# ooowedyn/InkLayer

Hardware: AMD Instinct MI355X
Metric: sketches/sec end-to-end (GroundingDINO+SAM) at 1024x1024 (higher is better)
Workload: dtype f16 (MFMA, f32 accumulate; f32 residual/norm/softmax; split-f16 = fp32-grade operands for patch-embed, neck, mask decoder); 1 GPU; full GroundingDINO Swin-T + SAM ViT-H pipeline, batch=8 per GPU, 1024x1024 synthetic sketches, 16 boxes/sketch, random-init weights; global_batch=8, parallelism=image-parallel x1

## Files before the change

inklayer_amd/csrc/attention.hip:

```cpp
#include <stdlib.h>
#include "mfma_util.h"
#include "../../include/inklayer_hip.h"

int ink_win4_attn_launch(const InkAttn& p, int n_cus, hipStream_t s);
int ink_glob4_attn_launch(const InkAttn& p, hipStream_t s);

namespace {

__device__ __forceinline__ f16x8 cvt8(const f32x16& s, int base) {
  f16x8 r;
#pragma unroll
  for (int j = 0; j < 8; ++j) r[j] = (f16)s[base + j];
  return r;
}

template <int HD, int MODE, int NW, bool ALLKV = false>
__global__ __launch_bounds__(NW * 64) void flash_attn_kernel(InkAttn p) {
  constexpr int NQKB = HD / 16;
  constexpr int NQK = NQKB + (MODE == 2 ? 2 : 0);
  constexpr int NB = (HD + 31) / 32;
  constexpr int DVP = NB * 32;
  constexpr bool LSUM_MFMA = DVP >= HD + 8;
  constexpr int CH = HD / 8;
  constexpr int KROW = ((NQK * 2) | 1) * 16;
// ... 319 lines not shown
    };
    if constexpr (LSUM_MFMA && !ALLKV) {
#pragma unroll
      for (int r = 0; r < 16; ++r) s0[r] = __builtin_amdgcn_exp2f(fmaf(s0[r], c, koff));
      pf[0] = cvt8(s0, 0);
      pf[1] = cvt8(s0, 8);
      if (half) {
#pragma unroll
        for (int ks = 0; ks < 2; ++ks)
#pragma unroll
          for (int i = 0; i < NB; ++i) pv(ks, i);
      } else {
        constexpr int NG = 2 * NB;
#pragma unroll
        for (int g = 0; g < NG; ++g) {
          pv(g / NB, g % NB);
#pragma unroll
          for (int r = (16 * g) / NG; r < (16 * (g + 1)) / NG; ++r) s1[r] = __builtin_amdgcn_exp2f(fmaf(s1[r], c, koff));
        }
        pf[2] = cvt8(s1, 0);
        pf[3] = cvt8(s1, 8);
#pragma unroll
        for (int ks = 2; ks < 4; ++ks)
#pragma unroll
          for (int i = 0; i < NB; ++i) pv(ks, i);
      }
    } else {
      float ps = 0.f;
#pragma unroll
      for (int r = 0; r < 16; ++r) {
        s0[r] = __builtin_amdgcn_exp2f(fmaf(s0[r], c, koff));
        s1[r] = __builtin_amdgcn_exp2f(fmaf(s1[r], c, koff));
        ps += s0[r] + s1[r];
      }
      if constexpr (!LSUM_MFMA) l_run += ps;
      pf[0] = cvt8(s0, 0);
      pf[1] = cvt8(s0, 8);
      pf[2] = cvt8(s1, 0);
      pf[3] = cvt8(s1, 8);
#pragma unroll
      for (int ks = 0; ks < 4; ++ks) {
        if (ks >= 2 && half) break;
#pragma unroll
        for (int i = 0; i < NB; ++i) pv(ks, i);
      }
    }
    if constexpr (!ALLKV) {
      if (t + 1 < ntiles) {
        store_tile(t + 1);
        if (t + 2 < ntiles) load_tile(t + 2);
      }
      __syncthreads();
    }
  }

  float ltot;
  if constexpr (LSUM_MFMA) {
    ltot = o[LI][LR];
  } else {
    ltot = l_run + __shfl_xor(l_run, 32, 64);
  }
  const float inv = 1.0f / ltot;
  if (q_ok) {
    const int64_t o_row = (MODE == 2 && ALLKV && p.tok_rows) ? q_row : (int64_t)b * p.n_q + q_idx;
    f16* Orow = (f16*)p.O + o_row * p.ldo + h * HD;
#pragma unroll
    for (int i = 0; i < NB; ++i)
#pragma unroll
      for (int g = 0; g < 4; ++g) {
        const int d0 = 32 * i + 8 * g + 4 * hh;
        if (d0 < HD) {
          const f16x4 v = {(f16)(o[i][4 * g] * inv), (f16)(o[i][4 * g + 1] * inv),
                           (f16)(o[i][4 * g + 2] * inv), (f16)(o[i][4 * g + 3] * inv)};
          *(f16x4*)(Orow + d0) = v;
        }
      }
  }
  if constexpr (ALLKV) {
    if (blk + 1 < blk_end) qs = load_q(blk + 1, qf);
  }
  }
}

template <int HD, int S, bool AUG, bool F16T = false>
__global__ __launch_bounds__(256) void relpos_mfma_kernel(const f16* __restrict__ Q, int64_t ldq,
                                                          const float* __restrict__ Rh,
                                                          const float* __restrict__ Rw, int n_heads,
                                                          float inv_scale, const int32_t* __restrict__ tok_rows,
                                                          float* __restrict__ out_h, float* __restrict__ out_w,
                                                          f16* __restrict__ out_aug) {
  constexpr int NQ = S * S;
  constexpr int RT = (2 * S - 1 + 31) / 32;
  constexpr int ROWS = 2 * RT * 32;
  constexpr int TROW = (HD / 8 + 1) * 16;
  constexpr int NQG = (NQ + 31) / 32;
  constexpr int GPB = AUG ? NQG : 8;
  constexpr int OROW = (AUG ? 64 : 256) + 16;
  __shared__ __attribute__((aligned(16))) char tab[ROWS * TROW + 4 * 32 * OROW];
  const int tid = threadIdx.x, lane = tid & 63, wave = tid >> 6;
  const int lq = lane & 31, hh = lane >> 5;
  char* ot = tab + ROWS * TROW + wave * 32 * OROW;
  const int nblk = (NQG + GPB - 1) / GPB;
  const int bh = blockIdx.x / nblk, gb = blockIdx.x % nblk;
  const int b = bh / n_heads, h = bh % n_heads;
  for (int i = tid; i < ROWS * (HD / 8); i += 256) {
    const int r = i / (HD / 8), c8 = i % (HD / 8);
    const int tr = r % (RT * 32);
    const float* src = (r < RT * 32 ? Rh : Rw) + (int64_t)tr * HD + c8 * 8;
    f16x8 v = {0, 0, 0, 0, 0, 0, 0, 0};
    if (tr < 2 * S - 1) {
      const f32x4 a = *(const f32x4*)src, c = *(const f32x4*)(src + 4);
      v = (f16x8){(f16)a[0], (f16)a[1], (f16)a[2], (f16)a[3], (f16)c[0], (f16)c[1], (f16)c[2], (f16)c[3]};
    }
    *(f16x8*)(tab + r * TROW + c8 * 16) = v;
  }
  __syncthreads();
  for (int g = gb * GPB + wave; g < min(NQG, (gb + 1) * GPB); g += 4) {
    const int q = g * 32 + lq;
    bool q_ok = q < NQ;
    const int qc = q_ok ? q : NQ - 1;
    int64_t qrow = (int64_t)b * NQ + qc;
    if (AUG && tok_rows) {
      const int r = tok_rows[qrow];
      q_ok = q_ok && r >= 0;
      qrow = r >= 0 ? r : 0;
    }
    const f16* qp = Q + qrow * ldq + h * HD;
    f16x8 qf[HD / 16];
#pragma unroll
    for (int s = 0; s < HD / 16; ++s) qf[s] = *(const f16x8*)(qp + 16 * s + 8 * hh);
    const int qh = qc / S, qw = qc % S;
    if (AUG && hh == 0) *(f16x4*)(ot + lq * OROW + 56) = (f16x4){0, 0, 0, 0};
#pragma unroll
    for (int tt = 0; tt < 2 * RT; ++tt) {
      f32x16 d;
#pragma unroll
      for (int r = 0; r < 16; ++r) d[r] = 0.f;
#pragma unroll
      for (int s = 0; s < HD / 16; ++s) {
        const f16x8 a = *(const f16x8*)(tab + (tt * 32 + lq) * TROW + (2 * s + hh) * 16);
        d = mfma32(a, qf[s], d);
      }
      const bool is_w = tt >= RT;
      const int base = (is_w ? qw : qh) + S - 1 - (tt % RT) * 32;
#pragma unroll
      for (int r = 0; r < 16; ++r) {
        const int j = base - ((r & 3) + 8 * (r >> 2) + 4 * hh);
        if (j >= 0 && j < S) {
          const float v = d[r] * inv_scale;
          if (AUG) {
            *(f16*)(ot + lq * OROW + ((is_w ? S : 0) + j) * 2) = (f16)v;
          } else {
            *(float*)(ot + lq * OROW + j * 4) = v;
          }
        }
      }
      if (!AUG && (tt % RT) == RT - 1) {
        if (F16T) {
          f16* dst = (f16*)(is_w ? out_w : out_h) + ((int64_t)bh * NQ + q) * S + hh * 32;
          if (q_ok) {
#pragma unroll
            for (int i = 0; i < 4; ++i) {
              const f32x4 a = *(const f32x4*)(ot + lq * OROW + hh * 128 + i * 32), c = *(const f32x4*)(ot + lq * OROW + hh * 128 + i * 32 + 16);
              *(f16x8*)(dst + 8 * i) = (f16x8){(f16)a[0], (f16)a[1], (f16)a[2], (f16)a[3], (f16)c[0], (f16)c[1], (f16)c[2], (f16)c[3]};
            }
          }
        } else {
          float* dst = (is_w ? out_w : out_h) + ((int64_t)bh * NQ + q) * S + hh * 32;
          if (q_ok) {
#pragma unroll
            for (int i = 0; i < 8; ++i) *(f32x4*)(dst + 4 * i) = *(const f32x4*)(ot + lq * OROW + hh * 128 + i * 16);
          }
        }
      }
    }
    if (AUG && q_ok) {
      f16* dst = out_aug + ((int64_t)bh * NQ + q) * 32 + hh * 16;
      *(f16x8*)dst = *(const f16x8*)(ot + lq * OROW + hh * 32);
      *(f16x8*)(dst + 8) = *(const f16x8*)(ot + lq * OROW + hh * 32 + 16);
    }
  }
}

}

extern "C" int ink_flash_attn(const InkAttn* pp, void* stream) {
  INK_CHECK_ARG(pp != nullptr);
  const InkAttn& p = *pp;
  INK_CHECK_ARG(p.Q && p.K && p.V && p.O);
  INK_CHECK_ARG(p.n_batch > 0 && p.n_heads > 0 && p.n_q > 0 && p.n_k > 0);
  INK_CHECK_ARG(p.ldq % 8 == 0 && p.ldk % 8 == 0 && p.ldv % 8 == 0 && p.ldo % 4 == 0);
  INK_CHECK_ARG(ink_aligned<16>(p.Q, p.K, p.V) && ink_aligned<8>(p.O));
  INK_CHECK_ARG(!p.tok_rows || p.bias_mode == 2);
  static const int n_cus = [] {
    int dev = 0, n = 0;
    if (hipGetDevice(&dev) != hipSuccess || hipDeviceGetAttribute(&n, hipDeviceAttributeMultiprocessorCount, dev) != hipSuccess || n <= 0) n = 256;
    return n;
  }();
  constexpr bool persist = true;
  hipStream_t s = (hipStream_t)stream;
  const int bhn = p.n_batch * p.n_heads;
#define INK_FA_X(HD, MODE, NW, ALL)                                                                      \
  {                                                                                                        \
    constexpr int nqk_ = HD / 16 + (MODE == 2 ? 2 : 0);                                                    \
    constexpr int lds_ = (ALL ? 4 : 2) * (64 * (((nqk_ * 2) | 1) * 16) + 64 * (((HD + 31) / 32) * 64)) +   \
                         0;                                                                            \
    ink_dyn_lds<flash_attn_kernel<HD, MODE, NW, ALL>>(lds_);                                               \
    const int nqb = (p.n_q + NW * 32 - 1) / (NW * 32);                                                     \
    const int grid_ = (ALL && persist) ? (bhn * nqb < n_cus ? bhn * nqb : n_cus) : bhn * nqb;                \
    hipLaunchKernelGGL((flash_attn_kernel<HD, MODE, NW, ALL>), dim3(grid_), dim3(NW * 64), lds_, s, p);      \
  }
#define INK_FA(HD, MODE, NW) INK_FA_X(HD, MODE, NW, false)
  if (p.head_dim == 80 && p.bias_mode == 1) {
    INK_CHECK_ARG(p.rel_h && p.rel_w && p.grid_w == 64 && p.n_k % 64 == 0);
    if (p.n_q % 256 == 0 && p.n_k % 128 == 0 && p.n_k >= 256 && p.n_k <= 4096) return ink_glob4_attn_launch(p, s);
    INK_CHECK_ARG(!p.rel_f16);
    INK_FA(80, 1, 8);
  } else if (p.head_dim == 80 && p.bias_mode == 2) {
    INK_CHECK_ARG(p.rel_aug && p.grid_w > 0 && p.grid_w <= 16 && p.n_k <= p.grid_w * p.grid_w && p.n_k <= 256);
    INK_CHECK_ARG(!p.tok_rows || (p.n_q == p.n_k && p.pad_k && p.pad_v &&
                                  ink_aligned<16>(p.pad_k, p.pad_v)));
    if (p.n_k >= 193 && p.n_k <= 208 && p.n_q <= 256 &&
        (p.tok_rows || (int64_t)p.n_batch * p.n_q * p.ldo * 2 < 0x80000000LL))
      return ink_win4_attn_launch(p, n_cus, s);
    INK_FA_X(80, 2, 7, true);
  } else if (p.head_dim == 64 && p.bias_mode == 1) {
    INK_CHECK_ARG(p.rel_h && p.rel_w && p.grid_w == 64 && p.n_k % 64 == 0 && p.n_k <= 64 * 64);
    INK_CHECK_ARG(!p.rel_f16);
    INK_FA(64, 1, 8);
  } else if (p.head_dim == 64 && p.bias_mode == 2) {
    INK_CHECK_ARG(p.rel_aug && p.grid_w > 0 && p.grid_w <= 16 && p.n_k <= p.grid_w * p.grid_w && p.n_k <= 256);
    INK_CHECK_ARG(!p.tok_rows || (p.n_q == p.n_k && p.pad_k && p.pad_v &&
                                  ink_aligned<16>(p.pad_k, p.pad_v)));
    INK_FA_X(64, 2, 7, true);
  } else if (p.head_dim == 80 && p.bias_mode == 0) {
    INK_FA(80, 0, 4);
  } else if (p.head_dim == 64 && p.bias_mode == 0) {
    INK_FA(64, 0, 4);
  } else if (p.head_dim == 32 && p.bias_mode == 0) {
    if (p.n_q <= 32) { INK_FA(32, 0, 1) } else { INK_FA(32, 0, 4) }
  } else if (p.head_dim == 32 && p.bias_mode == 3) {
    INK_CHECK_ARG(p.dense_bias && p.n_k <= 64 && p.n_q <= 64 && (!p.dense_mask || p.n_mask > 0));
    INK_FA(32, 3, 2);
  } else if (p.head_dim == 16 && p.bias_mode == 0) {
    if (p.n_q <= 32) { INK_FA(16, 0, 1) } else { INK_FA(16, 0, 4) }
  } else {
    return INK_ERR_ARG;
  }
#undef INK_FA
#undef INK_FA_X
  return ink_launch_status();
}

extern "C" int ink_relpos_bias64_f16(const void* Q, int64_t ldq, const float* rel_pos_h, const float* rel_pos_w,
                                     int32_t n_batch, int32_t n_heads, int32_t head_dim, float scale, void* out_h_f16,
                                     void* out_w_f16, void* stream) {
  INK_CHECK_ARG(Q && rel_pos_h && rel_pos_w && head_dim == 80 && ldq % 8 == 0 && out_h_f16 && out_w_f16);
  INK_CHECK_ARG(n_batch > 0 && n_heads > 0 && scale > 0.f && ink_aligned<16>(out_h_f16, out_w_f16));
  hipLaunchKernelGGL((relpos_mfma_kernel<80, 64, false, true>), dim3(n_batch * n_heads * 16), dim3(256), 0, (hipStream_t)stream,
                     (const f16*)Q, ldq, rel_pos_h, rel_pos_w, n_heads, 1.0f / scale, (const int32_t*)nullptr,
                     (float*)out_h_f16, (float*)out_w_f16, (f16*)nullptr);
  return ink_launch_status();
}

extern "C" int ink_relpos_bias(const void* Q, int64_t ldq, const float* rel_pos_h,
                               const float* rel_pos_w, int32_t S, int32_t n_batch,
                               int32_t n_heads, int32_t head_dim, float scale, const int32_t* tok_rows,
                               float* out_h, float* out_w, void* out_aug_f16, void* stream) {
  INK_CHECK_ARG(Q && rel_pos_h && rel_pos_w && (head_dim == 80 || head_dim == 64) && ldq % 8 == 0);
  INK_CHECK_ARG(n_batch > 0 && n_heads > 0 && S > 0 && scale > 0.f);
  if (out_aug_f16) {
    INK_CHECK_ARG(S <= 16);
  } else {
    INK_CHECK_ARG(S == 64 && out_h && out_w && !tok_rows);
  }
  const f16* q = (const f16*)Q;
  hipStream_t st = (hipStream_t)stream;
  const int nbh = n_batch * n_heads;
  if (out_aug_f16) {
    INK_CHECK_ARG(S == 14);
    if (head_dim == 80) {
      hipLaunchKernelGGL((relpos_mfma_kernel<80, 14, true>), dim3(nbh), dim3(256), 0, st, q, ldq, rel_pos_h,
                         rel_pos_w, n_heads, 1.0f / scale, tok_rows, out_h, out_w, (f16*)out_aug_f16);
    } else {
      hipLaunchKernelGGL((relpos_mfma_kernel<64, 14, true>), dim3(nbh), dim3(256), 0, st, q, ldq, rel_pos_h,
                         rel_pos_w, n_heads, 1.0f / scale, tok_rows, out_h, out_w, (f16*)out_aug_f16);
    }
  } else if (head_dim == 80) {
    hipLaunchKernelGGL((relpos_mfma_kernel<80, 64, false>), dim3(nbh * 16), dim3(256), 0, st, q, ldq, rel_pos_h,
                       rel_pos_w, n_heads, 1.0f / scale, (const int32_t*)nullptr, out_h, out_w, (f16*)nullptr);
  } else {
    hipLaunchKernelGGL((relpos_mfma_kernel<64, 64, false>), dim3(nbh * 16), dim3(256), 0, st, q, ldq, rel_pos_h,
                       rel_pos_w, n_heads, 1.0f / scale, (const int32_t*)nullptr, out_h, out_w, (f16*)nullptr);
  }
  return ink_launch_status();
}
```

inklayer_amd/csrc/attn_few.hip:

```cpp
#include "common.h"
#include "../../include/inklayer_hip.h"

namespace {

__device__ __forceinline__ void load8(const f16* p, float* d) {
  const f16x8 v = *(const f16x8*)p;
#pragma unroll
  for (int j = 0; j < 8; ++j) d[j] = (float)v[j];
}
__device__ __forceinline__ void load8(const float* p, float* d) {
  const f32x4 a = *(const f32x4*)p, b = *(const f32x4*)(p + 4);
#pragma unroll
  for (int j = 0; j < 4; ++j) { d[j] = a[j]; d[4 + j] = b[j]; }
}
__device__ __forceinline__ void store8(f16* p, const float* d) {
  f16x8 v;
#pragma unroll
  for (int j = 0; j < 8; ++j) v[j] = (f16)d[j];
  *(f16x8*)p = v;
}
__device__ __forceinline__ void store8(float* p, const float* d) {
  *(f32x4*)p = (f32x4){d[0], d[1], d[2], d[3]};
  *(f32x4*)(p + 4) = (f32x4){d[4], d[5], d[6], d[7]};
}

template <int HD, typename T>
__global__ __launch_bounds__(256) void attn_fewkeys_kernel(const T* __restrict__ Q, int64_t ldq,
                                                           const T* __restrict__ K, int64_t ldk,
                                                           const T* __restrict__ V, int64_t ldv, int B,
                                                           int n_q, int n_k, int n_heads, float scale,
                                                           const uint8_t* __restrict__ blocked,
                                                           const int32_t* __restrict__ q_rows,
                                                           const float* __restrict__ q_add,
                                                           T* __restrict__ O, int64_t ldo) {
  const int64_t gid = (int64_t)blockIdx.x * 256 + threadIdx.x;
  if (gid >= (int64_t)B * n_q * n_heads) return;
  const int h = (int)(gid % n_heads);
  const int64_t bq = gid / n_heads;
  const int b = (int)(bq / n_q), q = (int)(bq % n_q);
  float qv[HD];
  const T* qp = Q + (q_rows ? (int64_t)q_rows[b] + q : bq) * ldq + h * HD;
#pragma unroll
  for (int i = 0; i < HD / 8; ++i) load8(qp + 8 * i, qv + 8 * i);
  if (q_add) {
    const float* ap = q_add + ((int64_t)q * n_heads + h) * HD;
#pragma unroll
    for (int i = 0; i < HD; ++i) qv[i] += ap[i];
  }
  float sc[16];
  float mx = -3.0e38f;
  for (int t = 0; t < n_k; ++t) {
    const T* kp = K + ((int64_t)b * n_k + t) * ldk + h * HD;
    float d = 0.f;
#pragma unroll
    for (int i = 0; i < HD / 8; ++i) {
      float kv[8];
      load8(kp + 8 * i, kv);
#pragma unroll
      for (int j = 0; j < 8; ++j) d = fmaf(qv[8 * i + j], kv[j], d);
    }
    d *= scale;
    if (blocked && blocked[q * n_k + t]) d = -3.0e38f;
    sc[t] = d;
    mx = fmaxf(mx, d);
  }
  float sum = 0.f;
  for (int t = 0; t < n_k; ++t) { sc[t] = sc[t] <= -1.0e38f ? 0.f : expf(sc[t] - mx); sum += sc[t]; }
  const float inv = 1.f / sum;
  float acc[HD];
#pragma unroll
  for (int i = 0; i < HD; ++i) acc[i] = 0.f;
  for (int t = 0; t < n_k; ++t) {
    const T* vp = V + ((int64_t)b * n_k + t) * ldv + h * HD;
    const float pw = sc[t] * inv;
#pragma unroll
    for (int i = 0; i < HD / 8; ++i) {
      float vv[8];
      load8(vp + 8 * i, vv);
#pragma unroll
      for (int j = 0; j < 8; ++j) acc[8 * i + j] = fmaf(pw, vv[j], acc[8 * i + j]);
    }
  }
  T* op = O + bq * ldo + h * HD;
#pragma unroll
  for (int i = 0; i < HD / 8; ++i) store8(op + 8 * i, acc + 8 * i);
}


template <int NK>
__global__ __launch_bounds__(256) void attn_fewkeys16_f32_kernel(const float* __restrict__ Q, int64_t ldq,
                                                                 const float* __restrict__ K, int64_t ldk,
                                                                 const float* __restrict__ V, int64_t ldv, int B,
                                                                 int n_q, int n_heads, float scale,
                                                                 const int32_t* __restrict__ q_rows,
                                                                 const float* __restrict__ q_add,
                                                                 float* __restrict__ O, int64_t ldo) {
  const int64_t gid = (int64_t)blockIdx.x * 256 + threadIdx.x;
  if (gid >= (int64_t)B * n_q * n_heads * 4) return;
  const int part = (int)(gid & 3);
  const int h = (int)((gid >> 2) % n_heads);
  const int64_t bq = (gid >> 2) / n_heads;
  const int b = (int)(bq / n_q), q = (int)(bq % n_q);
  const int col = h * 16 + 4 * part;
  f32x4 qv = *(const f32x4*)(Q + (q_rows ? (int64_t)q_rows[b] + q : bq) * ldq + col);
  if (q_add) qv += *(const f32x4*)(q_add + (int64_t)q * n_heads * 16 + col);
  qv *= scale * 1.44269504088896340736f;
  const float* kp = K + (int64_t)b * NK * ldk + col;
  const float* vp = V + (int64_t)b * NK * ldv + col;
  f32x4 kv[NK], vv[NK];
#pragma unroll
  for (int t = 0; t < NK; ++t) {
    kv[t] = *(const f32x4*)(kp + (int64_t)t * ldk);
    vv[t] = *(const f32x4*)(vp + (int64_t)t * ldv);
  }
  float sc[NK];
  float mx = -3.0e38f;
#pragma unroll
  for (int t = 0; t < NK; ++t) {
    float d = (qv[0] * kv[t][0] + qv[1] * kv[t][1]) + (qv[2] * kv[t][2] + qv[3] * kv[t][3]);
    d += __builtin_bit_cast(float, __builtin_amdgcn_update_dpp(0, __builtin_bit_cast(int, d), 0xB1, 0xF, 0xF, false));
    d += __builtin_bit_cast(float, __builtin_amdgcn_update_dpp(0, __builtin_bit_cast(int, d), 0x4E, 0xF, 0xF, false));
    sc[t] = d;
    mx = fmaxf(mx, d);
  }
  float sum = 0.f;
#pragma unroll
  for (int t = 0; t < NK; ++t) { sc[t] = __builtin_amdgcn_exp2f(sc[t] - mx); sum += sc[t]; }
  const float inv = 1.f / sum;
  f32x4 acc = {0.f, 0.f, 0.f, 0.f};
#pragma unroll
  for (int t = 0; t < NK; ++t) acc += (sc[t] * inv) * vv[t];
  *(f32x4*)(O + bq * ldo + col) = acc;
}

template <int QW>
__global__ __launch_bounds__(512) void attn_fewq16_kernel(const float* __restrict__ Q, int64_t ldq,
                                                          const float* __restrict__ K, int64_t ldk,
                                                          const float* __restrict__ V, int64_t ldv, int n_q,
                                                          int n_k, int n_heads, float scale,
                                                          const int32_t* __restrict__ q_rows,
                                                          const int32_t* __restrict__ kv_rows,
                                                          const float* __restrict__ k_add,
                                                          float* __restrict__ O, int64_t ldo) {
  constexpr int KSPLIT = 2, HD = 16, HB = 4, TK = 64;
  constexpr int ROWE = HB * HD;
  constexpr int CH = 4, NCH = ROWE / CH;
  constexpr int NU = TK * NCH / 256;
  constexpr bool Q_IN_LDS = QW > 2;
  extern __shared__ __attribute__((aligned(16))) char fewq_smem[];
  const int grp = threadIdx.x >> 8;
  float* sk = (float*)fewq_smem + grp * 2 * TK * ROWE;
  float* sv = sk + TK * ROWE;
  const int hgroups = n_heads / HB;
  const int b = blockIdx.x / hgroups, h0 = (blockIdx.x % hgroups) * HB;
  const int tid = threadIdx.x & 255, lane = tid & 63, wave = tid >> 6;
  const int per = ((n_k + KSPLIT - 1) / KSPLIT + TK - 1) / TK * TK;
  const int k_lo = grp * per, k_hi = min(n_k, k_lo + per);
  const int kl = lane >> 2, hl = lane & 3;
  const int64_t q0 = q_rows ? (int64_t)q_rows[b] : (int64_t)b * n_q;
  const int64_t k0 = kv_rows ? (int64_t)kv_rows[b] : (int64_t)b * n_k;
  float* sq = (float*)fewq_smem + KSPLIT * 2 * TK * ROWE;
  float qr[QW][HD];
  if (!Q_IN_LDS || (grp == 0 && kl == 0)) {
    const float sc2 = scale * 1.44269504088896340736f;
#pragma unroll
    for (int j = 0; j < QW; ++j) {
      const int qi = QW * wave + j;
      const float* pq = Q + (q0 + (qi < n_q ? qi : 0)) * ldq + (h0 + hl) * HD;
      load8(pq, qr[j]);
      load8(pq + 8, qr[j] + 8);
#pragma unroll
      for (int e = 0; e < HD; ++e) qr[j][e] *= sc2;
      if constexpr (Q_IN_LDS) {
        store8(sq + (qi * HB + hl) * HD, qr[j]);
        store8(sq + (qi * HB + hl) * HD + 8, qr[j] + 8);
      }
    }
  }
  float m[QW], l[QW], acc[QW][HD];
#pragma unroll
  for (int j = 0; j < QW; ++j) {
    m[j] = -3.0e38f;
    l[j] = 0.f;
#pragma unroll
    for (int i = 0; i < HD; ++i) acc[j][i] = 0.f;
  }
  f32x4 rk[NU], rv[NU];
  auto fetch = [&](int t0) {
#pragma unroll
    for (int u = 0; u < NU; ++u) {
      const int c = tid + 256 * u, row = c / NCH, col = c % NCH;
      rk[u] = rv[u] = (f32x4){0.f, 0.f, 0.f, 0.f};
      if (t0 + row < k_hi) {
        rk[u] = *(const f32x4*)(K + (k0 + t0 + row) * ldk + h0 * HD + col * CH);
        rv[u] = *(const f32x4*)(V + (k0 + t0 + row) * ldv + h0 * HD + col * CH);
        if (k_add) rk[u] += *(const f32x4*)(k_add + (int64_t)(t0 + row) * n_heads * HD + h0 * HD + col * CH);
      }
    }
  };
  fetch(k_lo);
  for (int t0 = k_lo; t0 < k_lo + per; t0 += TK) {
    __syncthreads();
#pragma unroll
    for (int u = 0; u < NU; ++u) {
      const int c = tid + 256 * u, row = c / NCH, col = c % NCH;
      *(f32x4*)(sk + row * ROWE + col * CH) = rk[u];
      *(f32x4*)(sv + row * ROWE + col * CH) = rv[u];
    }
    __syncthreads();
    if (t0 + TK < k_hi) fetch(t0 + TK);
    float d[QW][TK / 16];
#pragma unroll
    for (int kk = 0; kk < TK / 16; ++kk) {
      const int key = kk * 16 + kl;
      float kf[HD];
// ... 44 lines not shown
        l[j] += pj;
#pragma unroll
        for (int e = 0; e < HD; ++e) acc[j][e] = fmaf(pj, vf[e], acc[j][e]);
      }
    }
  }
#pragma unroll
  for (int j = 0; j < QW; ++j) {
#pragma unroll
    for (int o = 4; o < 64; o <<= 1) {
      const float mo = __shfl_xor(m[j], o, 64), lo = __shfl_xor(l[j], o, 64);
      const float mn = fmaxf(m[j], mo);
      const float a = __builtin_amdgcn_exp2f(m[j] - mn), bsc = __builtin_amdgcn_exp2f(mo - mn);
      l[j] = l[j] * a + lo * bsc;
#pragma unroll
      for (int i = 0; i < HD; ++i) acc[j][i] = acc[j][i] * a + __shfl_xor(acc[j][i], o, 64) * bsc;
      m[j] = mn;
    }
  }
  __syncthreads();
  float* st = (float*)fewq_smem;
  if (grp > 0 && kl == 0) {
#pragma unroll
    for (int j = 0; j < QW; ++j) {
      float* ps = st + ((((grp - 1) * 4 + wave) * QW + j) * 4 + hl) * 18;
      ps[0] = m[j];
      ps[1] = l[j];
#pragma unroll
      for (int i = 0; i < HD; ++i) ps[2 + i] = acc[j][i];
    }
  }
  __syncthreads();
  if (grp > 0) return;
  if (kl == 0) {
#pragma unroll
    for (int g2 = 1; g2 < KSPLIT; ++g2)
#pragma unroll
      for (int j = 0; j < QW; ++j) {
        const float* ps = st + ((((g2 - 1) * 4 + wave) * QW + j) * 4 + hl) * 18;
        const float mo = ps[0], mn = fmaxf(m[j], mo);
        const float a = __builtin_amdgcn_exp2f(m[j] - mn), bsc = __builtin_amdgcn_exp2f(mo - mn);
        l[j] = l[j] * a + ps[1] * bsc;
#pragma unroll
        for (int i = 0; i < HD; ++i) acc[j][i] = acc[j][i] * a + ps[2 + i] * bsc;
        m[j] = mn;
      }
#pragma unroll
    for (int j = 0; j < QW; ++j) {
      const int qi = QW * wave + j;
      if (qi < n_q) {
        const float inv = 1.f / l[j];
#pragma unroll
        for (int i = 0; i < HD; ++i) acc[j][i] *= inv;
        float* op = O + ((int64_t)b * n_q + qi) * ldo + (h0 + hl) * HD;
        store8(op, acc[j]);
        store8(op + 8, acc[j] + 8);
      }
    }
  }
}

}

extern "C" int ink_attn_fewkeys(const void* Q, int64_t ldq, const void* K, int64_t ldk, const void* V,
                                int64_t ldv, int32_t B, int32_t n_q, int32_t n_k, int32_t n_heads,
                                int32_t head_dim, float scale, const uint8_t* blocked,
                                const int32_t* q_batch_rows, const float* q_add, int32_t io_f32, void* O,
                                int64_t ldo, void* stream) {
  INK_CHECK_ARG(Q && K && V && O && B > 0 && n_q > 0 && n_k > 0 && n_k <= 16 && n_heads > 0);
  INK_CHECK_ARG(ldq % 8 == 0 && ldk % 8 == 0 && ldv % 8 == 0 && ldo % 8 == 0);
  INK_CHECK_ARG(io_f32 == 0 || io_f32 == 1);
  INK_CHECK_ARG(ink_aligned<16>(Q, K, V, O, q_add));
  const int64_t total = (int64_t)B * n_q * n_heads;
  const dim3 grid((unsigned)((total + 255) / 256)), block(256);
  hipStream_t s = (hipStream_t)stream;
#define INK_FEWKEYS(HD, T)                                                                                     \
  hipLaunchKernelGGL((attn_fewkeys_kernel<HD, T>), grid, block, 0, s, (const T*)Q, ldq, (const T*)K, ldk,      \
                     (const T*)V, ldv, B, n_q, n_k, n_heads, scale, blocked, q_batch_rows, q_add, (T*)O, ldo)
  if (head_dim == 32 && !io_f32) INK_FEWKEYS(32, f16);
  else if (head_dim == 64 && !io_f32) INK_FEWKEYS(64, f16);
  else if (!io_f32) return INK_ERR_ARG;
  else if (head_dim == 32) INK_FEWKEYS(32, float);
  else if (head_dim == 16 && !blocked && n_k >= 7) {
    const dim3 g4((unsigned)((total * 4 + 255) / 256));
#define INK_FEWKEYS16(NK)                                                                                        \
  case NK:                                                                                                      \
    hipLaunchKernelGGL(attn_fewkeys16_f32_kernel<NK>, g4, block, 0, s, (const float*)Q, ldq, (const float*)K, ldk, \
                       (const float*)V, ldv, B, n_q, n_heads, scale, q_batch_rows, q_add, (float*)O, ldo);         \
    break
    switch (n_k) {
      INK_FEWKEYS16(7); INK_FEWKEYS16(8); INK_FEWKEYS16(9); INK_FEWKEYS16(10); INK_FEWKEYS16(11);
      INK_FEWKEYS16(12); INK_FEWKEYS16(13); INK_FEWKEYS16(14); INK_FEWKEYS16(15); INK_FEWKEYS16(16);
      default: return INK_ERR_ARG;
    }
#undef INK_FEWKEYS16
  } else if (head_dim == 16) INK_FEWKEYS(16, float);
  else return INK_ERR_ARG;
#undef INK_FEWKEYS
  return ink_launch_status();
}

extern "C" int ink_attn_fewq(const void* Q, int64_t ldq, const void* K, int64_t ldk, const void* V, int64_t ldv,
                             int32_t n_batch, int32_t n_q, int32_t n_k, int32_t n_heads, int32_t head_dim,
                             float scale, const int32_t* q_batch_rows, const int32_t* kv_batch_rows,
                             const float* k_add, void* O, int64_t ldo, void* stream) {
  INK_CHECK_ARG(Q && K && V && O && n_batch > 0 && n_q > 0 && n_q <= 16 && n_k > 0 && n_heads > 0);
  INK_CHECK_ARG(head_dim == 16 && n_heads % 4 == 0);
  INK_CHECK_ARG(ldq % 8 == 0 && ldk % 8 == 0 && ldv % 8 == 0 && ldo % 8 == 0);
  INK_CHECK_ARG(ink_aligned<16>(Q, K, V, O, k_add));
  constexpr int lds2 = 2 * 2 * 64 * 64 * 4, lds4 = lds2 + 16 * 64 * 4;
  ink_dyn_lds<attn_fewq16_kernel<2>>(lds2);
  ink_dyn_lds<attn_fewq16_kernel<4>>(lds4);
  const bool wide = n_q > 8;
  hipLaunchKernelGGL(wide ? attn_fewq16_kernel<4> : attn_fewq16_kernel<2>, dim3(n_batch * (n_heads / 4)), dim3(512),
                     wide ? lds4 : lds2, (hipStream_t)stream, (const float*)Q, ldq, (const float*)K, ldk,
                     (const float*)V, ldv, n_q, n_k, n_heads, scale, q_batch_rows, kv_batch_rows, k_add, (float*)O, ldo);
  return ink_launch_status();
}
```

inklayer_amd/csrc/sam_decoder.hip:

```cpp
#include "common.h"
#include "sam_postprocess.h"
#include "../../include/inklayer_hip.h"

namespace {

__device__ __forceinline__ void pe_feature(float x, float y, const float* __restrict__ G, int F, int f, float& sv,
                                           float& cv) {
  const float cx = 2.f * x - 1.f, cy = 2.f * y - 1.f;
  float v = cx * G[f] + cy * G[F + f];
  v = 6.283185307179586f * v;
  sv = sinf(v);
  cv = cosf(v);
}

__global__ __launch_bounds__(256) void pe_encode_kernel(const float* __restrict__ coords,
                                                        const float* __restrict__ G, int N, int F,
                                                        const float* __restrict__ add, int n_add,
                                                        float* __restrict__ out) {
  const int i = blockIdx.x * 256 + threadIdx.x;
  if (i >= N * F) return;
  const int n = i / F, f = i % F;
  float sv, cv;
  pe_feature(coords[2 * n], coords[2 * n + 1], G, F, f, sv, cv);
  if (add) {
// ... 169 lines not shown
  float acc = 0.f;
#pragma unroll
  for (int c = 0; c < C; c += 4) {
    const f32x4 uv = *(const f32x4*)(u + c);
    const f32x4 hv = *(const f32x4*)(h + c);
    acc = fmaf(hv[0], uv[0], acc);
    acc = fmaf(hv[1], uv[1], acc);
    acc = fmaf(hv[2], uv[2], acc);
    acc = fmaf(hv[3], uv[3], acc);
  }
  const int Y = 4 * y + 2 * (s1 >> 1) + (s2 >> 1), X = 4 * x + 2 * (s1 & 1) + (s2 & 1);
  out[((int64_t)b * 4 * g + Y) * 4 * g + X] = acc;
}

__global__ __launch_bounds__(256) void postprocess_kernel(const float* __restrict__ low, int n, int S,
                                                          int L, int in_h, int in_w, int out_h,
                                                          int out_w, float thr,
                                                          uint8_t* __restrict__ out,
                                                          float* __restrict__ out_logits) {
  const int64_t total = (int64_t)n * out_h * out_w;
  const PostScales sc = post_scales(S, L, in_h, in_w, out_h, out_w);
  for (int64_t i = (int64_t)blockIdx.x * 256 + threadIdx.x; i < total; i += (int64_t)gridDim.x * 256) {
    const int X = (int)(i % out_w), Y = (int)((i / out_w) % out_h);
    const int b = (int)(i / ((int64_t)out_w * out_h));
    const float v = post_pixel(low + (int64_t)b * S * S, S, sc, in_h, in_w, Y, X);
    if (out) out[i] = v > thr ? 1 : 0;
    if (out_logits) out_logits[i] = v;
  }
}

__global__ __launch_bounds__(256) void postprocess_rows_kernel(const float* __restrict__ low, int n, int S, int L,
                                                               int in_h, int in_w, int out_h, int out_w, float thr,
                                                               uint8_t* __restrict__ out,
                                                               float* __restrict__ out_logits) {
  constexpr int PX = 4;
  const float sA = (float)S / (float)L;
  const float sBh = (float)in_h / (float)out_h, sBw = (float)in_w / (float)out_w;
  const int wq = out_w / PX;
  for (int xq = threadIdx.x; xq < wq; xq += 256) {
    float lx[PX], lc[PX][2];
    int c0[PX][2], c1[PX][2];
#pragma unroll
    for (int px = 0; px < PX; ++px) {
      int x0, x1;
      bil(xq * PX + px, sBw, in_w, x0, x1, lx[px]);
      bil(x0, sA, S, c0[px][0], c1[px][0], lc[px][0]);
      bil(x1, sA, S, c0[px][1], c1[px][1], lc[px][1]);
    }
    for (int row = blockIdx.x; row < n * out_h; row += gridDim.x) {
      const int b = row / out_h, Y = row - b * out_h;
      const float* lp = low + (int64_t)b * S * S;
      int y0, y1;
      float ly;
      bil(Y, sBh, in_h, y0, y1, ly);
      int a0[2], a1[2];
      float la[2];
      bil(y0, sA, S, a0[0], a1[0], la[0]);
      bil(y1, sA, S, a0[1], a1[1], la[1]);
      const float* r00 = lp + a0[0] * S;
      const float* r01 = lp + a1[0] * S;
      const float* r10 = lp + a0[1] * S;
      const float* r11 = lp + a1[1] * S;
      float vals[PX];
#pragma unroll
      for (int px = 0; px < PX; ++px) {
        auto stageA = [&](const float* ra, const float* rb, float lav, int k) {
          const float v00 = ra[c0[px][k]], v01 = ra[c1[px][k]];
          const float v10 = rb[c0[px][k]], v11 = rb[c1[px][k]];
          return (1.f - lav) * ((1.f - lc[px][k]) * v00 + lc[px][k] * v01) + lav * ((1.f - lc[px][k]) * v10 + lc[px][k] * v11);
        };
        const float v00 = stageA(r00, r01, la[0], 0), v01 = stageA(r00, r01, la[0], 1);
        const float v10 = stageA(r10, r11, la[1], 0), v11 = stageA(r10, r11, la[1], 1);
        vals[px] = (1.f - ly) * ((1.f - lx[px]) * v00 + lx[px] * v01) + ly * ((1.f - lx[px]) * v10 + lx[px] * v11);
      }
      const int64_t o = (int64_t)row * out_w + (int64_t)xq * PX;
      if (out)
        *(uint32_t*)(out + o) = (uint32_t)(vals[0] > thr) | ((uint32_t)(vals[1] > thr) << 8) |
                                ((uint32_t)(vals[2] > thr) << 16) | ((uint32_t)(vals[3] > thr) << 24);
      if (out_logits) *(f32x4*)(out_logits + o) = (f32x4){vals[0], vals[1], vals[2], vals[3]};
    }
  }
}

}

extern "C" int ink_sam_pe_encode(const float* coords01, const float* gauss, int32_t N, int32_t F,
                                 const float* add, int32_t n_add, float* out, void* stream) {
  INK_CHECK_ARG(coords01 && gauss && out && N > 0 && F > 0 && (!add || n_add > 0));
  hipLaunchKernelGGL(pe_encode_kernel, dim3((N * F + 255) / 256), dim3(256), 0, (hipStream_t)stream,
                     coords01, gauss, N, F, add, n_add, out);
  return ink_launch_status();
}

extern "C" int ink_sam_mask_logits(const float* up, const float* hyper, int32_t n, int32_t g,
                                   int32_t C, float* out, void* stream) {
  INK_CHECK_ARG(up && hyper && out && n > 0 && g > 0);
  const int64_t total = (int64_t)n * g * g * 16;
  const dim3 grid((unsigned)((total + 255) / 256)), block(256);
  if (C == 32) {
    hipLaunchKernelGGL(mask_logits_kernel<32>, grid, block, 0, (hipStream_t)stream, up, hyper, n, g, out);
  } else if (C == 8) {
    hipLaunchKernelGGL(mask_logits_kernel<8>, grid, block, 0, (hipStream_t)stream, up, hyper, n, g, out);
  } else {
    return INK_ERR_ARG;
  }
  return ink_launch_status();
}

extern "C" int ink_sam_postprocess(const float* low, int32_t n, int32_t S, int32_t L, int32_t in_h,
                                   int32_t in_w, int32_t out_h, int32_t out_w, float thr,
                                   void* out_u8, float* out_logits, void* stream) {
  INK_CHECK_ARG(low && (out_u8 || out_logits) && n > 0 && S > 0 && L >= S);
  INK_CHECK_ARG(in_h > 0 && in_w > 0 && in_h <= L && in_w <= L && out_h > 0 && out_w > 0);
  const int64_t total = (int64_t)n * out_h * out_w;
  if (out_w % 4 == 0 && (int64_t)n * out_h < (int64_t)1 << 30 && ink_aligned<4>(out_u8) &&
      ink_aligned<16>(out_logits)) {
    const int64_t rows = (int64_t)n * out_h;
    const int blocks = (int)(rows < 8192 ? rows : 8192);
    hipLaunchKernelGGL(postprocess_rows_kernel, dim3(blocks), dim3(256), 0, (hipStream_t)stream, low, n, S, L, in_h,
                       in_w, out_h, out_w, thr, (uint8_t*)out_u8, out_logits);
    return ink_launch_status();
  }
  const int blocks = (int)((total + 255) / 256 < 16384 ? (total + 255) / 256 : 16384);
  hipLaunchKernelGGL(postprocess_kernel, dim3(blocks), dim3(256), 0, (hipStream_t)stream, low, n, S,
                     L, in_h, in_w, out_h, out_w, thr, (uint8_t*)out_u8, out_logits);
  return ink_launch_status();
}

extern "C" int ink_sam_prompt_tokens(const float* points, const int32_t* labels, int32_t n_pts, int32_t pad,
                                     const float* boxes, const float* gauss, int32_t F, const float* point_emb,
                                     const float* not_a_point, const float* out_tok, float input_size, int32_t P,
                                     float* out, void* stream) {
  INK_CHECK_ARG(gauss && point_emb && not_a_point && out_tok && out && P > 0 && F > 0 && input_size > 0.f);
  INK_CHECK_ARG(n_pts >= 0 && (n_pts == 0 || (points && labels)) && (pad == 0 || pad == 1));
  const int NT = 5 + n_pts + pad + (boxes ? 2 : 0);
  INK_CHECK_ARG(NT <= 16);
  const int64_t total = (int64_t)P * NT * F;
  hipLaunchKernelGGL(prompt_tokens_kernel, dim3((unsigned)((total + 255) / 256)), dim3(256), 0, (hipStream_t)stream,
                     points, labels, n_pts, pad, boxes, gauss, F, point_emb, not_a_point, out_tok, input_size, P, NT, out);
  return ink_launch_status();
}

extern "C" int ink_sam_mask_embed(const float* mask, const float* emb, const int32_t* emb_rows, const float* params,
                                  int32_t n_params, float eps, int32_t P, int32_t g, float* keys, void* split_f16,
                                  void* stream) {
  INK_CHECK_ARG(mask && emb && emb_rows && params && keys && P > 0 && g > 0 && g <= 64 && n_params == MP_TOTAL);
  INK_CHECK_ARG(ink_aligned<16>(mask, emb, keys) && ink_aligned<8>(split_f16));
  hipLaunchKernelGGL(mask_embed_kernel, dim3((unsigned)(P * g)), dim3(256), 0, (hipStream_t)stream, mask, emb, emb_rows,
                     params, eps, g, keys, (f16*)split_f16);
  return ink_launch_status();
}
```

Baseline: 118.7 sketches/s.

## Prefetch Q in relpos kernel, batch fewkeys16 pairs, add LDS postprocess kernel

The relpos MFMA kernel now processes more query groups per block and software-prefetches the next group's Q fragments while the current one computes, using fewer blocks. The few-keys head-dim-16 attention kernel gives each thread several query/head pairs and loads K/V once when the head index stays fixed, cutting redundant K/V loads. A new SAM mask postprocess kernel stages the low-res rows and a horizontally upsampled intermediate in LDS, with the next row prefetched into registers. These are three separate optimizations across unrelated kernels. Risks include more register pressure from prefetch buffers and fewer blocks for occupancy.

```diff
diff --git a/inklayer_amd/csrc/attention.hip b/inklayer_amd/csrc/attention.hip
--- a/inklayer_amd/csrc/attention.hip
+++ b/inklayer_amd/csrc/attention.hip
@@ -425,6 +425,7 @@
   }
 }
 
+constexpr int RELPOS_GPB_GLOB = 16;
 template <int HD, int S, bool AUG, bool F16T = false>
 __global__ __launch_bounds__(256) void relpos_mfma_kernel(const f16* __restrict__ Q, int64_t ldq,
                                                           const float* __restrict__ Rh,
@@ -437,7 +438,7 @@
   constexpr int ROWS = 2 * RT * 32;
   constexpr int TROW = (HD / 8 + 1) * 16;
   constexpr int NQG = (NQ + 31) / 32;
-  constexpr int GPB = AUG ? NQG : 8;
+  constexpr int GPB = AUG ? NQG : RELPOS_GPB_GLOB;
   constexpr int OROW = (AUG ? 64 : 256) + 16;
   __shared__ __attribute__((aligned(16))) char tab[ROWS * TROW + 4 * 32 * OROW];
   const int tid = threadIdx.x, lane = tid & 63, wave = tid >> 6;
@@ -446,6 +447,25 @@
   const int nblk = (NQG + GPB - 1) / GPB;
   const int bh = blockIdx.x / nblk, gb = blockIdx.x % nblk;
   const int b = bh / n_heads, h = bh % n_heads;
+  auto load_q = [&](int g, f16x8 (&dst)[HD / 16]) -> bool {
+    const int q = g * 32 + lq;
+    bool q_ok = q < NQ;
+    const int qc = q_ok ? q : NQ - 1;
+    int64_t qrow = (int64_t)b * NQ + qc;
+    if (AUG && tok_rows) {
+      const int r = tok_rows[qrow];
+      q_ok = q_ok && r >= 0;
+      qrow = r >= 0 ? r : 0;
+    }
+    const f16* qp = Q + qrow * ldq + h * HD;
+#pragma unroll
+    for (int s = 0; s < HD / 16; ++s) dst[s] = *(const f16x8*)(qp + 16 * s + 8 * hh);
+    return q_ok;
+  };
+  static_assert(AUG || (NQG % RELPOS_GPB_GLOB == 0 && RELPOS_GPB_GLOB % 4 == 0), "global form: whole blocks, whole rounds");
+  f16x8 qn[HD / 16];
+  bool okn = false;
+  if constexpr (!AUG) okn = load_q(gb * GPB + wave, qn);
   for (int i = tid; i < ROWS * (HD / 8); i += 256) {
     const int r = i / (HD / 8), c8 = i % (HD / 8);
     const int tr = r % (RT * 32);
@@ -458,20 +478,8 @@
     *(f16x8*)(tab + r * TROW + c8 * 16) = v;
   }
   __syncthreads();
-  for (int g = gb * GPB + wave; g < min(NQG, (gb + 1) * GPB); g += 4) {
-    const int q = g * 32 + lq;
-    bool q_ok = q < NQ;
-    const int qc = q_ok ? q : NQ - 1;
-    int64_t qrow = (int64_t)b * NQ + qc;
-    if (AUG && tok_rows) {
-      const int r = tok_rows[qrow];
-      q_ok = q_ok && r >= 0;
-      qrow = r >= 0 ? r : 0;
-    }
-    const f16* qp = Q + qrow * ldq + h * HD;
-    f16x8 qf[HD / 16];
-#pragma unroll
-    for (int s = 0; s < HD / 16; ++s) qf[s] = *(const f16x8*)(qp + 16 * s + 8 * hh);
+  auto group = [&](int q, bool q_ok, const f16x8 (&qf)[HD / 16]) {
+    const int qc = q < NQ ? q : NQ - 1;
     const int qh = qc / S, qw = qc % S;
     if (AUG && hh == 0) *(f16x4*)(ot + lq * OROW + 56) = (f16x4){0, 0, 0, 0};
 #pragma unroll
@@ -521,6 +529,24 @@
       f16* dst = out_aug + ((int64_t)bh * NQ + q) * 32 + hh * 16;
       *(f16x8*)dst = *(const f16x8*)(ot + lq * OROW + hh * 32);
       *(f16x8*)(dst + 8) = *(const f16x8*)(ot + lq * OROW + hh * 32 + 16);
+    }
+  };
+  if constexpr (AUG) {
+    for (int g = gb * GPB + wave; g < min(NQG, (gb + 1) * GPB); g += 4) {
+      f16x8 qf[HD / 16];
+      const bool q_ok = load_q(g, qf);
+      group(g * 32 + lq, q_ok, qf);
+    }
+  } else {
+#pragma unroll
+    for (int k = 0; k < GPB / 4; ++k) {
+      const int g = gb * GPB + wave + 4 * k;
+      f16x8 qf[HD / 16];
+#pragma unroll
+      for (int s = 0; s < HD / 16; ++s) qf[s] = qn[s];
+      const bool q_ok = okn;
+      if (k + 1 < GPB / 4) okn = load_q(g + 4, qn);
+      group(g * 32 + lq, q_ok, qf);
     }
   }
 }
@@ -600,7 +626,7 @@
                                      void* out_w_f16, void* stream) {
   INK_CHECK_ARG(Q && rel_pos_h && rel_pos_w && head_dim == 80 && ldq % 8 == 0 && out_h_f16 && out_w_f16);
   INK_CHECK_ARG(n_batch > 0 && n_heads > 0 && scale > 0.f && ink_aligned<16>(out_h_f16, out_w_f16));
-  hipLaunchKernelGGL((relpos_mfma_kernel<80, 64, false, true>), dim3(n_batch * n_heads * 16), dim3(256), 0, (hipStream_t)stream,
+  hipLaunchKernelGGL((relpos_mfma_kernel<80, 64, false, true>), dim3(n_batch * n_heads * (128 / RELPOS_GPB_GLOB)), dim3(256), 0, (hipStream_t)stream,
                      (const f16*)Q, ldq, rel_pos_h, rel_pos_w, n_heads, 1.0f / scale, (const int32_t*)nullptr,
                      (float*)out_h_f16, (float*)out_w_f16, (f16*)nullptr);
   return ink_launch_status();
@@ -630,10 +656,10 @@
                          rel_pos_w, n_heads, 1.0f / scale, tok_rows, out_h, out_w, (f16*)out_aug_f16);
     }
   } else if (head_dim == 80) {
-    hipLaunchKernelGGL((relpos_mfma_kernel<80, 64, false>), dim3(nbh * 16), dim3(256), 0, st, q, ldq, rel_pos_h,
+    hipLaunchKernelGGL((relpos_mfma_kernel<80, 64, false>), dim3(nbh * (128 / RELPOS_GPB_GLOB)), dim3(256), 0, st, q, ldq, rel_pos_h,
                        rel_pos_w, n_heads, 1.0f / scale, (const int32_t*)nullptr, out_h, out_w, (f16*)nullptr);
   } else {
-    hipLaunchKernelGGL((relpos_mfma_kernel<64, 64, false>), dim3(nbh * 16), dim3(256), 0, st, q, ldq, rel_pos_h,
+    hipLaunchKernelGGL((relpos_mfma_kernel<64, 64, false>), dim3(nbh * (128 / RELPOS_GPB_GLOB)), dim3(256), 0, st, q, ldq, rel_pos_h,
                        rel_pos_w, n_heads, 1.0f / scale, (const int32_t*)nullptr, out_h, out_w, (f16*)nullptr);
   }
   return ink_launch_status();
diff --git a/inklayer_amd/csrc/attn_few.hip b/inklayer_amd/csrc/attn_few.hip
--- a/inklayer_amd/csrc/attn_few.hip
+++ b/inklayer_amd/csrc/attn_few.hip
@@ -87,6 +87,7 @@
 }
 
 
+constexpr int FEWKEYS16_IT = 8;
 template <int NK>
 __global__ __launch_bounds__(256) void attn_fewkeys16_f32_kernel(const float* __restrict__ Q, int64_t ldq,
                                                                  const float* __restrict__ K, int64_t ldk,
@@ -95,42 +96,61 @@
                                                                  const int32_t* __restrict__ q_rows,
                                                                  const float* __restrict__ q_add,
                                                                  float* __restrict__ O, int64_t ldo) {
-  const int64_t gid = (int64_t)blockIdx.x * 256 + threadIdx.x;
-  if (gid >= (int64_t)B * n_q * n_heads * 4) return;
-  const int part = (int)(gid & 3);
-  const int h = (int)((gid >> 2) % n_heads);
-  const int64_t bq = (gid >> 2) / n_heads;
-  const int b = (int)(bq / n_q), q = (int)(bq % n_q);
-  const int col = h * 16 + 4 * part;
-  f32x4 qv = *(const f32x4*)(Q + (q_rows ? (int64_t)q_rows[b] + q : bq) * ldq + col);
-  if (q_add) qv += *(const f32x4*)(q_add + (int64_t)q * n_heads * 16 + col);
-  qv *= scale * 1.44269504088896340736f;
-  const float* kp = K + (int64_t)b * NK * ldk + col;
-  const float* vp = V + (int64_t)b * NK * ldv + col;
+  constexpr int IT = FEWKEYS16_IT;
+  const int pairs = n_q * n_heads;
+  const int nchunk = (pairs + 64 * IT - 1) / (64 * IT);
+  const int b = blockIdx.x / nchunk;
+  const int p0 = (blockIdx.x % nchunk) * 64 * IT + (threadIdx.x >> 2);
+  const int part = threadIdx.x & 3;
+  const bool same_head = 64 % n_heads == 0;
+  const int64_t qrow0 = q_rows ? (int64_t)q_rows[b] : (int64_t)b * n_q;
+  f32x4 qv[IT];
+#pragma unroll
+  for (int it = 0; it < IT; ++it) {
+    const int p = p0 + 64 * it;
+    if (p < pairs) {
+      const int q = p / n_heads, col = (p % n_heads) * 16 + 4 * part;
+      qv[it] = *(const f32x4*)(Q + (qrow0 + q) * ldq + col);
+      if (q_add) qv[it] += *(const f32x4*)(q_add + (int64_t)q * n_heads * 16 + col);
+    }
+  }
   f32x4 kv[NK], vv[NK];
-#pragma unroll
-  for (int t = 0; t < NK; ++t) {
-    kv[t] = *(const f32x4*)(kp + (int64_t)t * ldk);
-    vv[t] = *(const f32x4*)(vp + (int64_t)t * ldv);
-  }
-  float sc[NK];
-  float mx = -3.0e38f;
-#pragma unroll
-  for (int t = 0; t < NK; ++t) {
-    float d = (qv[0] * kv[t][0] + qv[1] * kv[t][1]) + (qv[2] * kv[t][2] + qv[3] * kv[t][3]);
-    d += __builtin_bit_cast(float, __builtin_amdgcn_update_dpp(0, __builtin_bit_cast(int, d), 0xB1, 0xF, 0xF, false));
-    d += __builtin_bit_cast(float, __builtin_amdgcn_update_dpp(0, __builtin_bit_cast(int, d), 0x4E, 0xF, 0xF, false));
-    sc[t] = d;
-    mx = fmaxf(mx, d);
-  }
-  float sum = 0.f;
-#pragma unroll
-  for (int t = 0; t < NK; ++t) { sc[t] = __builtin_amdgcn_exp2f(sc[t] - mx); sum += sc[t]; }
-  const float inv = 1.f / sum;
-  f32x4 acc = {0.f, 0.f, 0.f, 0.f};
-#pragma unroll
-  for (int t = 0; t < NK; ++t) acc += (sc[t] * inv) * vv[t];
-  *(f32x4*)(O + bq * ldo + col) = acc;
+  auto load_kv = [&](int col) {
+    const float* kp = K + (int64_t)b * NK * ldk + col;
+    const float* vp = V + (int64_t)b * NK * ldv + col;
+#pragma unroll
+    for (int t = 0; t < NK; ++t) {
+      kv[t] = *(const f32x4*)(kp + (int64_t)t * ldk);
+      vv[t] = *(const f32x4*)(vp + (int64_t)t * ldv);
+    }
+  };
+  if (same_head) load_kv((p0 % n_heads) * 16 + 4 * part);
+#pragma unroll
+  for (int it = 0; it < IT; ++it) {
+    const int p = p0 + 64 * it;
+    if (p >= pairs) break;
+    const int q = p / n_heads, col = (p % n_heads) * 16 + 4 * part;
+    if (!same_head) load_kv(col);
+    const f32x4 qs = qv[it] * (scale * 1.44269504088896340736f);
+    float sc[NK];
+    float mx = -3.0e38f;
+#pragma unroll
+    for (int t = 0; t < NK; ++t) {
+      float d = (qs[0] * kv[t][0] + qs[1] * kv[t][1]) + (qs[2] * kv[t][2] + qs[3] * kv[t][3]);
+      d += __builtin_bit_cast(float, __builtin_amdgcn_update_dpp(0, __builtin_bit_cast(int, d), 0xB1, 0xF, 0xF, false));
+      d += __builtin_bit_cast(float, __builtin_amdgcn_update_dpp(0, __builtin_bit_cast(int, d), 0x4E, 0xF, 0xF, false));
+      sc[t] = d;
+      mx = fmaxf(mx, d);
+    }
+    float sum = 0.f;
+#pragma unroll
+    for (int t = 0; t < NK; ++t) { sc[t] = __builtin_amdgcn_exp2f(sc[t] - mx); sum += sc[t]; }
+    const float inv = 1.f / sum;
+    f32x4 acc = {0.f, 0.f, 0.f, 0.f};
+#pragma unroll
+    for (int t = 0; t < NK; ++t) acc += (sc[t] * inv) * vv[t];
+    *(f32x4*)(O + ((int64_t)b * n_q + q) * ldo + col) = acc;
+  }
 }
 
 template <int QW>
@@ -341,7 +361,9 @@
   else if (!io_f32) return INK_ERR_ARG;
   else if (head_dim == 32) INK_FEWKEYS(32, float);
   else if (head_dim == 16 && !blocked && n_k >= 7) {
-    const dim3 g4((unsigned)((total * 4 + 255) / 256));
+    const int64_t nchunk = ((int64_t)n_q * n_heads + 64 * FEWKEYS16_IT - 1) / (64 * FEWKEYS16_IT);
+    INK_CHECK_ARG((int64_t)n_q * n_heads < (int64_t)1 << 30 && B * nchunk < (int64_t)1 << 31);
+    const dim3 g4((unsigned)(B * nchunk));
 #define INK_FEWKEYS16(NK)                                                                                        \
   case NK:                                                                                                      \
     hipLaunchKernelGGL(attn_fewkeys16_f32_kernel<NK>, g4, block, 0, s, (const float*)Q, ldq, (const float*)K, ldk, \
diff --git a/inklayer_amd/csrc/sam_decoder.hip b/inklayer_amd/csrc/sam_decoder.hip
--- a/inklayer_amd/csrc/sam_decoder.hip
+++ b/inklayer_amd/csrc/sam_decoder.hip
@@ -275,6 +275,88 @@
   }
 }
 
+template <int NC>
+__global__ __launch_bounds__(256) void postprocess_lds_kernel(const float* __restrict__ low, int n, int S, int L,
+                                                              int in_h, int in_w, int out_h, int out_w, float thr,
+                                                              uint8_t* __restrict__ out,
+                                                              float* __restrict__ out_logits) {
+  constexpr int PX = 4;
+  constexpr int W = NC * 64 + 16;
+  __shared__ float lowr[4][256];
+  __shared__ float stA[2][4 * W];
+  const float sA = (float)S / (float)L;
+  const float sBh = (float)in_h / (float)out_h, sBw = (float)in_w / (float)out_w;
+  const int tid = threadIdx.x;
+  const bool has_px = tid < out_w / PX;
+  float lx[PX];
+  int p0[PX], p1[PX];
+#pragma unroll
+  for (int px = 0; px < PX; ++px) {
+    int x0, x1;
+    bil(tid * PX + px, sBw, in_w, x0, x1, lx[px]);
+    p0[px] = (x0 & 3) * W + (x0 >> 2);
+    p1[px] = (x1 & 3) * W + (x1 >> 2);
+  }
+  float lc[NC];
+  int c0[NC], c1[NC];
+#pragma unroll
+  for (int j = 0; j < NC; ++j) bil(tid + 256 * j, sA, S, c0[j], c1[j], lc[j]);
+  const int rows = n * out_h;
+  struct RowW { float ly, la[2]; };
+  auto load_low = [&](int row, float (&v)[4]) -> RowW {
+    const int b = row / out_h, Y = row - b * out_h;
+    const float* lp = low + (int64_t)b * S * S;
+    RowW w;
+    int y0, y1, a0[2], a1[2];
+    bil(Y, sBh, in_h, y0, y1, w.ly);
+    bil(y0, sA, S, a0[0], a1[0], w.la[0]);
+    bil(y1, sA, S, a0[1], a1[1], w.la[1]);
+    if (tid < S) {
+      v[0] = lp[a0[0] * S + tid];
+      v[1] = lp[a1[0] * S + tid];
+      v[2] = lp[a0[1] * S + tid];
+      v[3] = lp[a1[1] * S + tid];
+    }
+    return w;
+  };
+  float nv[4] = {0.f, 0.f, 0.f, 0.f};
+  RowW nw = {0.f, {0.f, 0.f}};
+  if ((int)blockIdx.x < rows) nw = load_low(blockIdx.x, nv);
+  for (int row = blockIdx.x; row < rows; row += gridDim.x) {
+    const RowW w = nw;
+#pragma unroll
+    for (int k = 0; k < 4; ++k) lowr[k][tid] = nv[k];
+    __syncthreads();
+    if (row + (int)gridDim.x < rows) nw = load_low(row + gridDim.x, nv);
+#pragma unroll
+    for (int j = 0; j < NC; ++j) {
+      const int x = tid + 256 * j;
+#pragma unroll
+      for (int k = 0; k < 2; ++k) {
+        const float v00 = lowr[2 * k][c0[j]], v01 = lowr[2 * k][c1[j]];
+        const float v10 = lowr[2 * k + 1][c0[j]], v11 = lowr[2 * k + 1][c1[j]];
+        stA[k][(x & 3) * W + (x >> 2)] =
+            (1.f - w.la[k]) * ((1.f - lc[j]) * v00 + lc[j] * v01) + w.la[k] * ((1.f - lc[j]) * v10 + lc[j] * v11);
+      }
+    }
+    __syncthreads();
+    if (has_px) {
+      float vals[PX];
+#pragma unroll
+      for (int px = 0; px < PX; ++px) {
+        const float v00 = stA[0][p0[px]], v01 = stA[0][p1[px]];
+        const float v10 = stA[1][p0[px]], v11 = stA[1][p1[px]];
+        vals[px] = (1.f - w.ly) * ((1.f - lx[px]) * v00 + lx[px] * v01) + w.ly * ((1.f - lx[px]) * v10 + lx[px] * v11);
+      }
+      const int64_t o = (int64_t)row * out_w + (int64_t)tid * PX;
+      if (out)
+        *(uint32_t*)(out + o) = (uint32_t)(vals[0] > thr) | ((uint32_t)(vals[1] > thr) << 8) |
+                                ((uint32_t)(vals[2] > thr) << 16) | ((uint32_t)(vals[3] > thr) << 24);
+      if (out_logits) *(f32x4*)(out_logits + o) = (f32x4){vals[0], vals[1], vals[2], vals[3]};
+    }
+  }
+}
+
 }
 
 extern "C" int ink_sam_pe_encode(const float* coords01, const float* gauss, int32_t N, int32_t F,
@@ -310,6 +392,19 @@
       ink_aligned<16>(out_logits)) {
     const int64_t rows = (int64_t)n * out_h;
     const int blocks = (int)(rows < 8192 ? rows : 8192);
+    if (S <= 256 && in_w <= 1024 && out_w <= 1024) {
+#define INK_POST(NC)                                                                                            \
+  hipLaunchKernelGGL(postprocess_lds_kernel<NC>, dim3(blocks), dim3(256), 0, (hipStream_t)stream, low, n, S, L, \
+                     in_h, in_w, out_h, out_w, thr, (uint8_t*)out_u8, out_logits)
+      switch ((in_w + 255) / 256) {
+        case 1: INK_POST(1); break;
+        case 2: INK_POST(2); break;
+        case 3: INK_POST(3); break;
+        default: INK_POST(4); break;
+      }
+#undef INK_POST
+      return ink_launch_status();
+    }
     hipLaunchKernelGGL(postprocess_rows_kernel, dim3(blocks), dim3(256), 0, (hipStream_t)stream, low, n, S, L, in_h,
                        in_w, out_h, out_w, thr, (uint8_t*)out_u8, out_logits);
     return ink_launch_status();
```

Result: no change. 119.3 sketches/s, median of 6 (+0.5%).
